# thomasneff/AdaNeRF

Measured on AMD Instinct MI355X. Metric: FPS at 800x800, higher is better.
Workload: dtype bf16

## Files before the change

### adanerf_amd/csrc/adanerf_hip.hip

```cpp
#include "../../include/adanerf_hip.h"

#include <hip/hip_runtime.h>

#include <sys/stat.h>

#include <algorithm>
#include <type_traits>
#include <cmath>
#include <cstdio>
#include <cstring>
#include <exception>
#include <string>
#include <vector>

#include "format.hpp"
#include "kernels.hip.hpp"
#include "launch_f32.hpp"
#include "k_generic_f32.hip.hpp"
#include "k_generic16.hip.hpp"
#include "pack.hpp"

using namespace adanerf;

namespace {
// ... 76 lines not shown
  int sample16_grid = 0;
  int sampling_mode = 0;
  DevBuf overflow;
  int sample_grid = 0;
  PackedDev net1[3];
  TensorMap net1_host;
  DevBuf ztab;
  bool coarse_fine = false;
  int n_coarse = 0;
  PackedDev netc[3];
  NetTopology topoc;
  bool genericc = false;
  GenericTopo genc{};
  ShadeParams spc{};
  DevBuf ztab_coarse, raw_coarse, key_coarse;
  int shade_gen_grid_c = 0;

  int cap_rays = 0, cap_nmax = 0;
  DevBuf rays, oracle, ray_offsets, ray_counts, selbin, selw, block_total, block_offset, total;
  DevBuf sample_key, sample_w, raw, sample_z;
  DevBuf guard_mask, refine_list, guard_probe;
  float guard_eps = 0.f;
  float guard_eps_pair = 0.f;
  int guard_audit_period = 0;
  DepthMap dm{};
  int shade_grid[3] = {0, 0, 0};
  int device = 0;
  float* aux_depth = nullptr;
  float* aux_acc = nullptr;
  float* aux_disp = nullptr;
  DevBuf disp_scratch;
  hipEvent_t peer_event = nullptr;
  uint64_t peer_tried = 0;
};

namespace {

#define HIP_TRY(ctx, expr)                                                                  \
  do {                                                                                      \
    hipError_t e_ = (expr);                                                                 \
    if (e_ != hipSuccess) {                                                                 \
      (ctx)->err = std::string(#expr) + ": " + hipGetErrorString(e_);                       \
      return ADANERF_EDEVICE;                                                               \
    }                                                                                       \
  } while (0)

#define BIND(ctx) HIP_TRY(ctx, hipSetDevice((ctx)->device))

int fail(adanerf_ctx* c, int code, const std::string& msg) {
  if (c) c->err = msg;
  else g_create_error = msg;
  return code;
}

int dev_alloc(adanerf_ctx* c, DevBuf* b, size_t bytes) {
  if (b->bytes >= bytes && b->p) return ADANERF_OK;
  if (b->p) HIP_TRY(c, hipFree(b->p));
  b->p = nullptr;
  b->bytes = 0;
  if (bytes == 0) return ADANERF_OK;
  HIP_TRY(c, hipMalloc(&b->p, bytes));
  b->bytes = bytes;
  return ADANERF_OK;
}

void dev_free(DevBuf* b) {
  if (b->p) (void)hipFree(b->p);
  b->p = nullptr;
  b->bytes = 0;
}

int upload_net(adanerf_ctx* c, const PackedNet& pn, PackedDev* d) {
  int rc;
  if ((rc = dev_alloc(c, &d->w, pn.weights.size()))) return rc;
  if ((rc = dev_alloc(c, &d->b, pn.bias.size() * sizeof(float)))) return rc;
  HIP_TRY(c, hipMemcpy(d->w.p, pn.weights.data(), pn.weights.size(), hipMemcpyHostToDevice));
  HIP_TRY(c, hipMemcpy(d->b.p, pn.bias.data(), pn.bias.size() * sizeof(float), hipMemcpyHostToDevice));
  d->params.w = reinterpret_cast<const u32x4*>(d->w.p);
  d->params.bias = reinterpret_cast<const float*>(d->b.p);
  for (size_t i = 0; i < pn.w_off.size() && i < kMaxLayers; ++i) {
// ... 381 lines not shown
template <typename K>
int occupancy_grid(adanerf_ctx* c, K kernel, int threads, int* out) {
  int per_cu = 0;
  HIP_TRY(c, hipOccupancyMaxActiveBlocksPerMultiprocessor(&per_cu, kernel, threads, 0));
  if (per_cu < 1) per_cu = 1;
  *out = per_cu * c->info.compute_units;
  return ADANERF_OK;
}

int calibrate_guard(adanerf_ctx* c, int n_poses, uint32_t seed, bool install, float* max_diff, float* max_pair);
int ensure_guard_band(adanerf_ctx* c);

bool has_split_sampling(const adanerf_ctx* c) { return (!c->generic0 || c->ray_samples == 0) && c->topo0.width != kWideWidth; }

bool generic_split_sampling(const adanerf_ctx* c) {
  return c->generic0 && c->sampling_mode != ADANERF_SAMPLING_FP32 && c->ray_samples == 0 && c->net0_split.w.p != nullptr;
}

int launch_sample_mlp(adanerf_ctx* c, int first_ray, int n_rays, float* d_oracle, float* d_rays, const SelectOut* sel = nullptr) {
  if (n_rays <= 0) return ADANERF_OK;
  SampleArgs a{};
  if (sel) {
    a.sel = *sel;
    a.fused_select = 1;
  }
  a.g = c->rg;
  a.net = c->net0.params;
  a.net16 = c->net0_split.params;
  a.overflow_flag = reinterpret_cast<int32_t*>(c->overflow.p);
  a.first_ray = first_ray;
  a.n_rays = n_rays;
  a.oracle_out = d_oracle;
  a.rays_out = d_rays;
  dim3 grid((n_rays + 127) / 128), block(256);
  const bool full = c->fp0 == 10 && c->fd0 == 4;
  if (c->generic0) {
    if (generic_split_sampling(c)) {
      const uint32_t bias_cap = c->topo0.width == 64 ? gen_bias_cap<64>() : c->topo0.width == 128 ? gen_bias_cap<128>() : gen_bias_cap<256>();
      if (tune::kGenericStaged && a.net16.n_bias > bias_cap)
        return fail(c, ADANERF_EUNSUPPORTED, "sampling network: bias table exceeds the kernel's LDS capacity");
#define ADN_GENS(FPv, FDv, Wv) hipLaunchKernelGGL((sample_mlp16x3_gen_kernel<FPv, FDv, Wv, tune::kGenericStaged>), grid, block, 0, c->stream, a, c->gen0)
#define ADN_GENS_W(FPv, FDv)                                   \
  do {                                                         \
    if (c->topo0.width == 64) ADN_GENS(FPv, FDv, 64);          \
    else if (c->topo0.width == 128) ADN_GENS(FPv, FDv, 128);   \
    else ADN_GENS(FPv, FDv, 256);                              \
  } while (0)
      if (c->enc0 == kEnc10_4) ADN_GENS_W(10, 4);
      else if (c->enc0 == kEnc2_2) ADN_GENS_W(2, 2);
      else ADN_GENS_W(kMaxBands, kMaxBands);
#undef ADN_GENS_W
#undef ADN_GENS
      HIP_TRY(c, hipGetLastError());
      return ADANERF_OK;
    }
    if (sel) return fail(c, ADANERF_EINVAL, "fused selection is not available on the fp32 run-time-shaped sampling kernel");
    HIP_TRY(c, launch_sample_mlp_gen(a, c->gen0, c->enc0, c->topo0.width, grid.x, c->stream));
    return ADANERF_OK;
  }
  const bool guarded = c->sampling_mode == ADANERF_SAMPLING_GUARDED && sel != nullptr;
  if (guarded) {
    if (!(c->guard_eps > 0.f)) {
      int rc = ensure_guard_band(c);
      if (rc) return rc;
    }
    a.sel.guard_mask = reinterpret_cast<uint32_t*>(c->guard_mask.p);
// ... 1 lines not shown
    a.sel.guard_pair = guard_pair_of(c->transform, c->guard_eps, c->guard_eps_pair);
    a.sel.audit_period = c->guard_audit_period;
    a.sel.audit_phase = c->guard_audit_period > 0 ? static_cast<int32_t>(c->guard_frame & static_cast<uint32_t>(c->guard_audit_period - 1)) : 0;
    a.sel.guard_probe = reinterpret_cast<float*>(c->guard_probe.p);
    a.sel.guard_rows = reinterpret_cast<float*>(c->oracle.p);
    if (c->debug_guard & 1) a.sel.guard_rows = nullptr;
    a.sel.guard_seen = reinterpret_cast<uint32_t*>(c->total.p) + 8;
  }
  if (c->sampling_mode == 1) {
    HIP_TRY(c, launch_sample_mlp_f32(a, full, grid.x, c->stream));
  } else if (c->sampling_mode == 2 || guarded) {
    if (!c->net0_f16.w.p) {
      PackedNet pn;
      std::string err;
      const NetShape sh = shape_of(c->fp0, c->fd0, c->fp1, c->fd1, c->ray_samples);
      if (!pack_sampling_net(c->net0_host, sh, Elem::F16, &pn, &err)) return fail(c, ADANERF_EIO, "model0.onnx: " + err);
      int rc = upload_net(c, pn, &c->net0_f16);
      if (rc) return rc;
    }
    a.net16 = c->net0_f16.params;
    if (!c->sample16_grid) {
      int rc = full ? occupancy_grid(c, sample_mlp16_kernel<10, 4>, 512, &c->sample16_grid)
                    : occupancy_grid(c, sample_mlp16_kernel<2, 2>, 512, &c->sample16_grid);
      if (rc) return rc;
    }
    const bool two_blocks = sel != nullptr && a.fused_select && !a.oracle_out && !(c->debug_guard & 2) && (n_rays >= kSample16x2MinRays || (c->debug_guard & 4));
    if (two_blocks) {
      if (!c->sample16x2_grid) {
        int rc = full ? occupancy_grid(c, sample_mlp16x2_kernel<10, 4>, 256, &c->sample16x2_grid)
                      : occupancy_grid(c, sample_mlp16x2_kernel<2, 2>, 256, &c->sample16x2_grid);
        if (rc) return rc;
      }
      dim3 g2(std::min<unsigned>((n_rays + 255) / 256, static_cast<unsigned>(c->sample16x2_grid))), b2(256);
      if (full) hipLaunchKernelGGL((sample_mlp16x2_kernel<10, 4>), g2, b2, 0, c->stream, a);
      else hipLaunchKernelGGL((sample_mlp16x2_kernel<2, 2>), g2, b2, 0, c->stream, a);
    } else {
    dim3 g16(std::min<unsigned>((n_rays + 255) / 256, static_cast<unsigned>(c->sample16_grid))), b16(512);
    if (full) hipLaunchKernelGGL((sample_mlp16_kernel<10, 4>), g16, b16, 0, c->stream, a);
    else hipLaunchKernelGGL((sample_mlp16_kernel<2, 2>), g16, b16, 0, c->stream, a);
    }
    if (guarded) {
      const int n_words = (n_rays + 31) / 32;
      int32_t* n_list = reinterpret_cast<int32_t*>(c->total.p) + 4;
      if (!c->sample_grid) {
        int rc = full ? occupancy_grid(c, sample_mlp16x3_kernel<10, 4>, 256, &c->sample_grid)
                      : occupancy_grid(c, sample_mlp16x3_kernel<2, 2>, 256, &c->sample_grid);
        if (rc) return rc;
      }
      const dim3 rgrid(std::min<unsigned>(grid.x, static_cast<unsigned>(c->sample_grid)));
      const int cap_round = (c->opt.flags & ADANERF_FLAG_GUARD_AUDIT_FILL) ? static_cast<int>(rgrid.x) * 128 : 0;
      const int cycle = a.sel.audit_period > 0 ? static_cast<int>((c->guard_frame / static_cast<uint32_t>(a.sel.audit_period)) & 0x7fffffffu) : 0;
      hipLaunchKernelGGL(refine_list_kernel, dim3((n_words + 255) / 256), dim3(256), 0, c->stream, reinterpret_cast<const uint32_t*>(c->guard_mask.p),
                         n_words, n_rays, a.sel.audit_period, a.sel.audit_phase, cap_round, cycle, reinterpret_cast<int32_t*>(c->refine_list.p), n_list);
      SampleArgs r = a;
      r.net16 = c->net0_split.params;
      r.rays_out = nullptr;
      r.sel.guard_mask = nullptr;
      r.sel.guard_band = c->guard_eps;
      r.sel.guard_band_pair = c->transform == kOracleRaw ? a.sel.guard_pair : 0.f;
      r.sel.guard_eps = 0.f;
      r.sel.guard_pair = 0.f;
      r.sel.audit_period = 0;
      r.sel.refine_list = reinterpret_cast<const int32_t*>(c->refine_list.p);
      r.ray_list = r.sel.refine_list;
      r.n_list = n_list;
      if (full) hipLaunchKernelGGL((sample_mlp16x3_kernel<10, 4>), rgrid, block, 0, c->stream, r);
      else hipLaunchKernelGGL((sample_mlp16x3_kernel<2, 2>), rgrid, block, 0, c->stream, r);
    }
  } else {
    if (!c->sample_grid) {
      int rc = full ? occupancy_grid(c, sample_mlp16x3_kernel<10, 4>, 256, &c->sample_grid)
                    : occupancy_grid(c, sample_mlp16x3_kernel<2, 2>, 256, &c->sample_grid);
      if (rc) return rc;
    }
    grid.x = std::min<unsigned>(grid.x, static_cast<unsigned>(c->sample_grid));
    if (full) hipLaunchKernelGGL((sample_mlp16x3_kernel<10, 4>), grid, block, 0, c->stream, a);
    else hipLaunchKernelGGL((sample_mlp16x3_kernel<2, 2>), grid, block, 0, c->stream, a);
  }
  HIP_TRY(c, hipGetLastError());
  return ADANERF_OK;
}

constexpr int kInlineScanMaxBlocks = 65536;

SelectOut select_out(adanerf_ctx* c, int n_max, float thr, int32_t* d_cnt) {
  SelectOut so{};
  so.counts = d_cnt;
  so.selbin = reinterpret_cast<uint8_t*>(c->selbin.p);
  so.selw = reinterpret_cast<float*>(c->selw.p);
  so.seg_total = reinterpret_cast<int32_t*>(c->block_total.p);
  so.n_max = n_max;
  so.thr = thr;
  so.transform = c->transform;
  return so;
}

int launch_expand(adanerf_ctx* c, int n_rays, int n_max, int seg_shift, int32_t* d_off, const int32_t* d_cnt, uint32_t* d_key, float* d_w,
                  int32_t* d_total) {
// ... 249 lines not shown
  return done(ADANERF_OK);
}

int ensure_guard_band(adanerf_ctx* c) {
  GuardRecord r;
  if (!(c->opt.flags & ADANERF_FLAG_NO_GUARD_CACHE) && read_guard_record(c, &r) && r.poses >= ADANERF_GUARD_CALIB_POSES) {
    install_guard_band(c, r.max_diff, r.max_pair, r.poses, ADANERF_GUARD_FROM_RECORD);
    return ADANERF_OK;
  }
  float d = 0.f, dp = 0.f;
  return calibrate_guard(c, ADANERF_GUARD_CALIB_POSES, 1u, true, &d, &dp);
}

constexpr int kShadeWaves = 8;

int launch_shade_mlp(adanerf_ctx* c, const float* d_rays, const uint32_t* d_key, const int32_t* d_total, int max_samples, int prec,
                     float* d_raw, const float* d_z = nullptr, bool coarse = false) {
  if (max_samples <= 0) return ADANERF_OK;
  const bool generic = coarse ? c->genericc : c->generic1;
  const NetTopology& topo = coarse ? c->topoc : c->topo1;
  const GenericTopo& gen = coarse ? c->genc : c->gen1;
  int& gen_grid = coarse ? c->shade_gen_grid_c : c->shade_gen_grid;
  int rc = coarse ? ensure_netc(c, prec) : ensure_net1(c, prec);
  if (rc) return rc;
  ShadeArgs a{};
  a.sp = coarse ? c->spc : c->sp;
  a.net = coarse ? c->netc[prec].params : c->net1[prec].params;
  a.rays = d_rays;
  a.sample_key = d_key;
  a.sample_z = d_z;
  a.total = d_total;
  a.max_samples = max_samples;
  a.raw_out = d_raw;
  if (generic && prec != ADANERF_PREC_FP32) {
    const int enc = coarse ? enc_layout(c->fp0, c->fd0, false) : c->enc1;
    const bool st = tune::kGenericStaged;
    const bool enc104 = enc == kEnc10_4;
    const int nb_wg = !st ? 1 : topo.width == 64 ? gen_blocks<64>() : topo.width == 128 ? (enc104 ? gen_blocks<128, 10>() : gen_blocks<128, kMaxBands>())
                                : topo.width == 256 ? gen_blocks<256>() : gen_blocks<512>();
    const int per_wg = 128 * nb_wg;
    const int tiles = (max_samples + per_wg - 1) / per_wg;
    const uint32_t bias_cap = topo.width == 64 ? gen_bias_cap<64>() : topo.width == 128 ? gen_bias_cap<128>()
                              : topo.width == 256 ? gen_bias_cap<256>() : gen_bias_cap<512>();
    if (st && a.net.n_bias > bias_cap)
      return fail(c, ADANERF_EUNSUPPORTED, "shading network: bias table exceeds the kernel's LDS capacity");
    int& grid16 = c->shade_gen16_grid[coarse ? 1 : 0][prec == ADANERF_PREC_BF16 ? 0 : 1];
#define ADN_GEN16_GO(KERNEL)                                                                                             \
  do {                                                                                                                   \
    if (!grid16) {                                                                                                       \
      int per_cu = 0;                                                                                                    \
      HIP_TRY(c, hipOccupancyMaxActiveBlocksPerMultiprocessor(&per_cu, KERNEL, 256, 0));                                 \
      grid16 = (per_cu < 1 ? 1 : per_cu) * c->info.compute_units;                                                        \
    }                                                                                                                    \
    hipLaunchKernelGGL(KERNEL, dim3(std::min(tiles, grid16)), dim3(256), 0, c->stream, a, gen);                          \
  } while (0)
#define ADN_GEN16(ET, FPv, FDv, Wv)                                                                                      \
  do {                                                                                                                   \
    if constexpr (tune::kGenericStaged)                                                                                  \
      ADN_GEN16_GO((shade_mlp16_gen_staged_kernel<ET, FPv, FDv, Wv, gen_blocks<Wv, FPv>(), gen_occupancy<Wv, FPv>()>));       \
    else ADN_GEN16_GO((shade_mlp16_gen_kernel<ET, FPv, FDv, Wv>));                                                       \
  } while (0)
#define ADN_GEN16_W(ET, FPv, FDv)                                  \
  do {                                                             \
    if (topo.width == 64) ADN_GEN16(ET, FPv, FDv, 64);             \
    else if (topo.width == 128) ADN_GEN16(ET, FPv, FDv, 128);      \
    else if (topo.width == 256) ADN_GEN16(ET, FPv, FDv, 256);      \
// ... 198 lines not shown
  c->guard_eps = opt->guard_eps > 0.f ? opt->guard_eps : 0.f;
  c->guard_eps_pair = (c->guard_eps > 0.f && opt->guard_eps_pair > 0.f) ? std::min(opt->guard_eps_pair, 2.0f * c->guard_eps) : 2.0f * c->guard_eps;
  c->guard_audit_period = opt->guard_audit_period == 0 ? ADANERF_GUARD_AUDIT_PERIOD : std::max(opt->guard_audit_period, 0);
  c->info.guard_eps = c->guard_eps;
  c->info.guard_eps_pair = c->guard_eps_pair;
  c->info.guard_audit_period = c->sampling_mode == ADANERF_SAMPLING_GUARDED ? c->guard_audit_period : 0;
  c->info.guard_calib_source = c->guard_eps > 0.f ? ADANERF_GUARD_FROM_OPTIONS : ADANERF_GUARD_FROM_NONE;
  if (c->sampling_mode == ADANERF_SAMPLING_GUARDED) c->model0_hash = fnv1a64_file(join_path(model_dir, "model0.onnx"));
  {
    PackedNet probe;
    if (!pack_shading_net(c->net1_host, sh, Elem::F32, &probe, &err)) return bail(ADANERF_EIO, "model1.onnx: " + err);
    c->topo1 = probe.topo;
    c->generic1 = !probe.topo.is_default(true) || c->enc1 == kEncMax;
    if (opt->precision == ADANERF_PREC_FP32) p1 = std::move(probe);
    else if (!pack_shading_net(c->net1_host, sh, elem_of(opt->precision), &p1, &err)) return bail(ADANERF_EIO, "model1.onnx: " + err);
  }
  auto width_ok = [](int w) { return w == 64 || w == 128 || w == 256 || w == kWideWidth; };
  if (c->genericc && !width_ok(c->topoc.width)) return bail(ADANERF_EUNSUPPORTED, "model0.onnx: layer width " + std::to_string(c->topoc.width) + " (64, 128, 256 or 512 supported)");
  if (c->generic0 && !width_ok(c->topo0.width)) return bail(ADANERF_EUNSUPPORTED, "model0.onnx: layer width " + std::to_string(c->topo0.width) + " (64, 128, 256 or 512 supported)");
  if (c->generic1 && !width_ok(c->topo1.width)) return bail(ADANERF_EUNSUPPORTED, "model1.onnx: layer width " + std::to_string(c->topo1.width) + " (64, 128, 256 or 512 supported)");

  int n_dev = 0;
  if (hipGetDeviceCount(&n_dev) != hipSuccess || n_dev <= 0)
    return bail(ADANERF_EDEVICE, "no HIP device available: libadanerf_hip has no CPU fallback");
  if (hipSetDevice(opt->device_id) != hipSuccess) return bail(ADANERF_EDEVICE, "hipSetDevice failed");
  hipDeviceProp_t prop;
  if (hipGetDeviceProperties(&prop, opt->device_id) != hipSuccess) return bail(ADANERF_EDEVICE, "hipGetDeviceProperties failed");
  if (std::string(prop.gcnArchName).find("gfx950") == std::string::npos)
    return bail(ADANERF_EDEVICE, std::string("device is ") + prop.gcnArchName + "; this library is built for gfx950 (MI355X) only");
  c->info.compute_units = prop.multiProcessorCount;
  c->device = opt->device_id;
  if (hipStreamCreateWithFlags(&c->own_stream, hipStreamNonBlocking) != hipSuccess) return bail(ADANERF_EDEVICE, "hipStreamCreate failed");
  c->stream = c->own_stream;

  rc = dev_alloc(c, &c->ztab, kBins * sizeof(float));
  if (rc) return bail(rc, c->err);
  if (hipMemcpy(c->ztab.p, ms.ztab.data(), kBins * sizeof(float), hipMemcpyHostToDevice) != hipSuccess)
    return bail(ADANERF_EDEVICE, "ztab upload failed");
  c->sp.ztab = reinterpret_cast<const float*>(c->ztab.p);
  if (c->coarse_fine) {
    if ((rc = upload_net(c, p0, &c->netc[opt->precision]))) return bail(rc, c->err);
    if ((rc = dev_alloc(c, &c->ztab_coarse, kMaxCoarse * sizeof(float)))) return bail(rc, c->err);
    if (hipMemcpy(c->ztab_coarse.p, ms.ztab_coarse.data(), ms.ztab_coarse.size() * sizeof(float), hipMemcpyHostToDevice) != hipSuccess)
      return bail(ADANERF_EDEVICE, "coarse depth table upload failed");
    c->spc = c->sp;
    c->spc.normalize = ms.normalize0;
    c->sp.unit_dir = 0;
    c->spc.ztab = reinterpret_cast<const float*>(c->ztab_coarse.p);
    c->genc = GenericTopo{c->topoc.depth, c->topoc.cat_mask, 0, 0, nullptr, 0.f};
  } else {
    if ((rc = upload_net(c, p0, &c->net0))) return bail(rc, c->err);
    if (has_split_sampling(c) && (rc = upload_net(c, p0s, &c->net0_split))) return bail(rc, c->err);
  }
  if (c->ray_samples > 0) {
    if ((rc = dev_alloc(c, &c->rsi_z, ms.rsi_z.size() * sizeof(float)))) return bail(rc, c->err);
    if (hipMemcpy(c->rsi_z.p, ms.rsi_z.data(), ms.rsi_z.size() * sizeof(float), hipMemcpyHostToDevice) != hipSuccess)
      return bail(ADANERF_EDEVICE, "raySampleInput depth table upload failed");
  }
  c->gen0 = GenericTopo{c->topo0.depth, 0, c->ray_samples, p0.rsi_w_off, reinterpret_cast<const float*>(c->rsi_z.p), c->cfg.depthRange[1]};
  c->gen1 = GenericTopo{c->topo1.depth, c->topo1.cat_mask, 0, 0, nullptr, 0.f};
  if ((rc = dev_alloc(c, &c->overflow, 64))) return bail(rc, c->err);
  if (hipMemset(c->overflow.p, 0, 64) != hipSuccess) return bail(ADANERF_EDEVICE, "hipMemset failed");
  if ((rc = upload_net(c, p1, &c->net1[opt->precision]))) return bail(rc, c->err);
  if ((rc = ensure_batch_buffers(c, c->info.batch_rays, c->info.num_samples))) return bail(rc, c->err);
  *out = c;
  return ADANERF_OK;
// ... 70 lines not shown
      layer_out[4 * i + 1] = pn.topo.ray_samples;
      layer_out[4 * i + 2] = pe_slots(sh.lp0 ? sh.lp0 : sh.fp0);
      layer_out[4 * i + 3] = pn.mtiles[0];
    }
    if (scaled) {
      const size_t i = pn.w_off.size();
      layer_out[4 * i + 0] = pn.out_exp[0];
      layer_out[4 * i + 1] = pn.out_exp[1];
      layer_out[4 * i + 2] = 0;
      layer_out[4 * i + 3] = -1;
    }
  }
  *weights_bytes = pn.weights.size();
  *bias_floats = pn.bias.size();
  *n_layers = n_rec;
  return ADANERF_OK;
} catch (const std::exception& e) {
  return fail(nullptr, ADANERF_EIO, std::string("adanerf_host_pack_weights: ") + e.what());
}

int adanerf_destroy(adanerf_ctx* c) {
  if (!c) return ADANERF_OK;
  (void)hipSetDevice(c->device);
  if (c->peer_event) (void)hipEventDestroy(c->peer_event);
  if (c->stream) (void)hipStreamSynchronize(c->stream);
  for (hipEvent_t e : c->events) (void)hipEventDestroy(e);
  for (int32_t* p : c->pinned_totals) (void)hipHostFree(p);
  if (c->guard_host) (void)hipHostFree(c->guard_host);
  if (c->guard_ev) (void)hipEventDestroy(c->guard_ev);
  DevBuf* bufs[] = {&c->net0_split.w, &c->net0_split.b, &c->net0_f16.w, &c->net0_f16.b, &c->overflow, &c->net0.w, &c->net0.b, &c->net1[0].w, &c->net1[0].b, &c->net1[1].w, &c->net1[1].b, &c->net1[2].w, &c->net1[2].b,
                    &c->ztab, &c->rays, &c->oracle, &c->ray_offsets, &c->ray_counts, &c->selbin, &c->selw, &c->block_total,
                    &c->block_offset, &c->total, &c->sample_key, &c->sample_w, &c->raw, &c->sample_z, &c->rsi_z,
                    &c->netc[0].w, &c->netc[0].b, &c->netc[1].w, &c->netc[1].b, &c->netc[2].w, &c->netc[2].b, &c->ztab_coarse, &c->raw_coarse, &c->key_coarse,
                    &c->guard_mask, &c->refine_list, &c->guard_probe, &c->disp_scratch};
  for (DevBuf* b : bufs) dev_free(b);
  if (c->own_stream) (void)hipStreamDestroy(c->own_stream);
  delete c;
  return ADANERF_OK;
}

int adanerf_get_info(const adanerf_ctx* c, adanerf_info* info) {
  if (!c || !info) return ADANERF_EINVAL;
  *info = c->info;
  return ADANERF_OK;
}

int adanerf_set_camera(adanerf_ctx* c, const float pos[3], const float rot[9]) {
  if (!c) return ADANERF_EINVAL;
  if (!pos || !rot) return fail(c, ADANERF_EINVAL, "pos/rot == NULL");
  if (c->pos_bound.active) {
    double d2 = 0.0;
    for (int i = 0; i < 3; ++i) d2 += (pos[i] - c->pos_bound.center[i]) * (pos[i] - c->pos_bound.center[i]);
    const double bound = c->pos_bound.at(std::sqrt(d2));
    if (!(bound <= kPosIdentityBound)) {
      char msg[256];
      std::snprintf(msg, sizeof(msg), "camera %.3g away from the view-cell centre: sample positions can reach %.3g, beyond the %.0f the bf16 shading path's "
                    "layer scaling assumes -- create the context with precision fp16 or fp32 for such poses", std::sqrt(d2), bound, kPosIdentityBound);
      return fail(c, ADANERF_EUNSUPPORTED, msg);
    }
  }
  std::memcpy(c->rg.pos, pos, 3 * sizeof(float));
  std::memcpy(c->rg.rot, rot, 9 * sizeof(float));
  return ADANERF_OK;
}

int adanerf_sync(adanerf_ctx* c) {
  if (!c) return ADANERF_EINVAL;
// ... 626 lines not shown
```

### adanerf_amd/csrc/k_mlp16.hip.hpp

```cpp
#pragma once
#include "k_common.hip.hpp"
#include "k_mlp_f32.hip.hpp"
#include "tuning.hpp"
#include <utility>

namespace adanerf {


struct ShadeArgs {
  ShadeParams sp;
  NetParams net;
  const float* rays;
  const uint32_t* sample_key;
  const float* sample_z;
  const int32_t* total;
  int32_t max_samples;
  float* raw_out;
};

__device__ __forceinline__ void store_raw(const ShadeArgs& a, int s, float r, float g, float b, float alpha) {
  const float ks = a.net.out_scale[1];
  *reinterpret_cast<float4*>(a.raw_out + static_cast<size_t>(s) * 4) = make_float4(r * ks, g * ks, b * ks, alpha * a.net.out_scale[0]);
}

struct Bf16 {
  static constexpr bool kClampRelu = true;
  typedef bf16x8 vec8;
  static __device__ __forceinline__ uint32_t pack(float lo, float hi) {
    f32x2 v = {lo, hi};
    return __builtin_bit_cast(uint32_t, __builtin_convertvector(v, bf16x2));
  }
  static __device__ __forceinline__ f32x16 mfma(u32x4 a, u32x4 b, f32x16 c) {
    return __builtin_amdgcn_mfma_f32_32x32x16_bf16(__builtin_bit_cast(bf16x8, a), __builtin_bit_cast(bf16x8, b), c, 0, 0, 0);
  }
};
struct Fp16 {
  static constexpr bool kClampRelu = false;
  typedef f16x8 vec8;
  static __device__ __forceinline__ uint32_t pack(float lo, float hi) {
    f32x2 v = {lo, hi};
    return __builtin_bit_cast(uint32_t, __builtin_convertvector(v, f16x2));
  }
  static __device__ __forceinline__ f32x16 mfma(u32x4 a, u32x4 b, f32x16 c) {
    return __builtin_amdgcn_mfma_f32_32x32x16_f16(__builtin_bit_cast(f16x8, a), __builtin_bit_cast(f16x8, b), c, 0, 0, 0);
  }
};

using tune::kRegFrags;
constexpr int kShadeFrags16 = 32 + 4 * 128 + 160 + 2 * 128 + 144 + 72 + 8;
constexpr int kShadeBiasFloats = 8 * 256 + 288 + 128 + 32;
// ... 496 lines not shown
      if (CARRY_OUT && kCarry) {
        pend.a = accA;
        pend.b = accB;
      } else {
        gA = mfma_guard<ET, RELU>(accA);
        gB = mfma_guard<ET, RELU>(accB);
#pragma unroll
        for (int g = 0; g < 4; ++g) epilogue_quad_16<ET, RELU>(accA, m, g, outA, gA);
#pragma unroll
        for (int g = 0; g < 4; ++g) epilogue_quad_16<ET, RELU>(accB, m, g, outB, gB);
      }
    }
  }
}

template <class ET, int FP, int FD>
__global__ __launch_bounds__(256) void shade_mlp16x2_kernel(ShadeArgs a) {
  static_assert(FP == 10 && FD == 4, "fragment positions below assume the 10-4 shading encoding");
  constexpr int QP = pe_slots(FP), QD = pe_slots(FD);
  constexpr int WAVES = 4, TILE = WAVES * 64, CF = tune::kChunkFrags2, RS = tune::kRingSlots2, LPW = CF / WAVES;
  constexpr int kRingBytes = CF * RS * 1024;
  static_assert(CF % WAVES == 0 && CF % tune::kRegFrags2 == 0 && kShadeFrags16 % CF == 0 && CF % 8 == 0 && CF <= 32, "chunk geometry");
  typedef WStream<CF, RS, LPW, tune::kRegFrags2> WS;
  constexpr int kStashPerBlock = (QP / 8 + QD / 8) * 1024;
  __shared__ __attribute__((aligned(16))) char lds[kRingBytes + kShadeBiasFloats * 4 + WAVES * 2 * kStashPerBlock];
  const int lane = lane_id();
  const int wave = __builtin_amdgcn_readfirstlane(static_cast<int>(threadIdx.x) >> 6);
  const int j = lane & 31, h = lane >> 5;
  const uint32_t stash = static_cast<uint32_t>(reinterpret_cast<uintptr_t>(lds)) + kRingBytes + kShadeBiasFloats * 4 +
                         wave * 2 * kStashPerBlock + lane * 16;
  int total = a.total ? *a.total : a.max_samples;
  if (total > a.max_samples) total = a.max_samples;
  const int ntiles = (total + TILE - 1) / TILE;
  if (static_cast<int>(blockIdx.x) >= ntiles) return;
  {
    float* lds_bias = reinterpret_cast<float*>(lds + kRingBytes);
    for (int i = threadIdx.x; i < kShadeBiasFloats; i += blockDim.x) lds_bias[i] = a.net.bias[i];
  }
  __syncthreads();
  WS st;
  ws_start(st, a.net.w, kShadeFrags16 * 1024, lds, wave, lane);
  const uint32_t bias0 = static_cast<uint32_t>(reinterpret_cast<uintptr_t>(lds)) + kRingBytes + h * 64;
  const uint32_t* bo = a.net.b_off;
  for (int tile = blockIdx.x; tile < ntiles; tile += gridDim.x) {
    const int s0 = tile * TILE + wave * 64 + j, s1 = s0 + 32;
    uint32_t hA0[64], hB0[64], hA1[64], hB1[64];
    PendingTile2 pend;
    {
      float x[3], dpe[3];
      uint32_t pts0[QP / 2], pts1[QP / 2], dirs[QD / 2];
      load_sample(a, s0, total, x, dpe);
      pe_pack<ET, FP>(x, h, pts0);
      pe_pack<ET, FD>(dpe, h, dirs);
      lds_stash_write<QP / 8>(stash, pts0);
      lds_stash_write<QD / 8>(stash + (QP / 8) * 1024, dirs);
      load_sample(a, s1, total, x, dpe);
      pe_pack<ET, FP>(x, h, pts1);
      pe_pack<ET, FD>(dpe, h, dirs);
      lds_stash_write<QP / 8>(stash + kStashPerBlock, pts1);
      lds_stash_write<QD / 8>(stash + kStashPerBlock + (QP / 8) * 1024, dirs);
      layer_16x2<ET, WS, QP / 8, 0, 8, true, 0, -1, -1, true, true>(st, bias0 + bo[0] * 4, pts0, pts0, pts1, pts1, hA0, hA1, pend);
    }
#pragma unroll 1
    for (int l = 1; l <= 3; l += 2) {
      layer_16x2<ET, WS, 16, 0, 8, true, 0, -1, 7, true, true>(st, bias0 + bo[l] * 4, hA0, hA0, hA1, hA1, hB0, hB1, pend, hA0, hA1);
      layer_16x2<ET, WS, 16, 0, 8, true, 0, -1, 7, true, true>(st, bias0 + bo[l + 1] * 4, hB0, hB0, hB1, hB1, hA0, hA1, pend, hB0, hB1);
    }
    {
      uint32_t pts0[QP / 2], pts1[QP / 2];
      lds_stash_read<QP / 8>(stash, pts0);
      lds_stash_read<QP / 8>(stash + kStashPerBlock, pts1);
      layer_16x2<ET, WS, QP / 8, 16, 8, true, 0, -1, 7, true, true>(st, bias0 + bo[5] * 4, pts0, hA0, pts1, hA1, hB0, hB1, pend, hA0, hA1);
    }
    layer_16x2<ET, WS, 16, 0, 8, true, 0, -1, 7, true, true>(st, bias0 + bo[6] * 4, hB0, hB0, hB1, hB1, hA0, hA1, pend, hB0, hB1);
    layer_16x2<ET, WS, 16, 0, 8, true, 0, -1, 7, true, true>(st, bias0 + bo[7] * 4, hA0, hA0, hA1, hA1, hB0, hB1, pend, hA0, hA1);
    f32x16 alpha0, alpha1;
    layer_16x2<ET, WS, 16, 0, 9, false, 0, 8, 7, true, false>(st, bias0 + bo[8] * 4, hB0, hB0, hB1, hB1, hA0, hA1, pend, hB0, hB1, &alpha0, &alpha1);
    {
      uint32_t d0[QD / 2], d1[QD / 2];
      lds_stash_read<QD / 8>(stash + (QP / 8) * 1024, d0);
      lds_stash_read<QD / 8>(stash + kStashPerBlock + (QP / 8) * 1024, d1);
      layer_16x2<ET, WS, 16, QD / 8, 4, true, (32 + 4 * 128 + 160 + 2 * 128 + 144) % CF>(st, bias0 + bo[9] * 4, hA0, d0, hA1, d1, hB0, hB1, pend);
    }
    f32x16 rgb0, rgb1;
    layer_16x2<ET, WS, 8, 0, 1, false, (32 + 4 * 128 + 160 + 2 * 128 + 144 + 72) % CF, 0>(st, bias0 + bo[10] * 4, hB0, hB0, hB1, hB1, hA0, hA1, pend, nullptr, nullptr, &rgb0, &rgb1);
    if (h == 0 && s0 < total)
      store_raw(a, s0, rgb0[0], rgb0[1], rgb0[2], alpha0[0]);
    if (h == 0 && s1 < total)
      store_raw(a, s1, rgb1[0], rgb1[1], rgb1[2], alpha1[0]);
  }
  asm volatile("s_waitcnt vmcnt(0)" ::: "memory");
}

template <int FP, int FD>
__global__ __launch_bounds__(256) void shade_mlp32_kernel(ShadeArgs a) {
  constexpr int QP = pe_slots(FP), QD = pe_slots(FD);
  constexpr int TILE = 4 * 32;
  const int lane = lane_id();
  const int wave = __builtin_amdgcn_readfirstlane(static_cast<int>(threadIdx.x) >> 6);
  const int j = lane & 31, h = lane >> 5;
  int total = a.total ? *a.total : a.max_samples;
  if (total > a.max_samples) total = a.max_samples;
  const u32x4* w = a.net.w;
  const float* b = a.net.bias;

  for (int tile = blockIdx.x; tile * TILE < total; tile += gridDim.x) {
    const int s = tile * TILE + wave * 32 + j;
    if (tile * TILE + wave * 32 >= total) continue;
    asm volatile("" : "+v"(w), "+v"(b));
    float x[3], dpe[3];
    load_sample(a, s, total, x, dpe);
    float pts[QP], dirs[QD], hA[144], hB[128];
    pe_eval<FP, true>(x, h, pts);
    pe_eval<FD, true>(dpe, h, dirs);
    layer_f32<QP, 0, 8, true>(w + a.net.w_off[0], b + a.net.b_off[0], lane, pts, pts, hA);
#pragma unroll 1
    for (int l = 1; l <= 3; l += 2) {
      layer_f32<128, 0, 8, true>(w + a.net.w_off[l], b + a.net.b_off[l], lane, hA, hA, hB);
      layer_f32<128, 0, 8, true>(w + a.net.w_off[l + 1], b + a.net.b_off[l + 1], lane, hB, hB, hA);
    }
    layer_f32<QP, 128, 8, true>(w + a.net.w_off[5], b + a.net.b_off[5], lane, pts, hA, hB);
    layer_f32<128, 0, 8, true>(w + a.net.w_off[6], b + a.net.b_off[6], lane, hB, hB, hA);
    layer_f32<128, 0, 8, true>(w + a.net.w_off[7], b + a.net.b_off[7], lane, hA, hA, hB);
// ... 39 lines not shown
```

### adanerf_amd/csrc/k_mlp_f32.hip.hpp

```cpp
#pragma once
#include "k_common.hip.hpp"
#include "k_select_pair.hip.hpp"

namespace adanerf {


template <int Q1, int Q2, int MT, bool RELU>
__device__ __forceinline__ void layer_f32(const u32x4* __restrict__ w, const float* __restrict__ bias, int lane,
                                          const float* in1, const float* in2, float* out) {
  constexpr int QS = Q1 + Q2;
  static_assert(Q1 % 4 == 0 && Q2 % 4 == 0, "fp32 engine groups 4 k-steps per 16-byte fragment");
  const int h = lane >> 5;
#pragma unroll
  for (int m = 0; m < MT; ++m) {
    f32x16 acc;
    const float4* bp = reinterpret_cast<const float4*>(bias + (m * 2 + h) * 16);
#pragma unroll
    for (int g = 0; g < 4; ++g) {
      float4 b = bp[g];
      acc[4 * g + 0] = b.x;
      acc[4 * g + 1] = b.y;
      acc[4 * g + 2] = b.z;
      acc[4 * g + 3] = b.w;
    }
#pragma unroll
    for (int s4 = 0; s4 < QS / 4; ++s4) {
      const f32x4 a = reinterpret_cast<const f32x4*>(w)[(m * (QS / 4) + s4) * 64 + lane];
      const float* in = (4 * s4 < Q1) ? (in1 + 4 * s4) : (in2 + (4 * s4 - Q1));
      acc = __builtin_amdgcn_mfma_f32_32x32x2f32(a[0], in[0], acc, 0, 0, 0);
      acc = __builtin_amdgcn_mfma_f32_32x32x2f32(a[1], in[1], acc, 0, 0, 0);
      acc = __builtin_amdgcn_mfma_f32_32x32x2f32(a[2], in[2], acc, 0, 0, 0);
      acc = __builtin_amdgcn_mfma_f32_32x32x2f32(a[3], in[3], acc, 0, 0, 0);
    }
#pragma unroll
    for (int r = 0; r < 16; ++r) out[16 * m + r] = RELU ? fmaxf(acc[r], 0.f) : acc[r];
  }
}

struct SampleArgs {
  RayGenParams g;
  NetParams net;
  NetParams net16;
  int32_t* overflow_flag;
  int32_t first_ray, n_rays;
  float* oracle_out;
  float* rays_out;
  SelectOut sel;
  int32_t fused_select;
  const int32_t* ray_list;
  const int32_t* n_list;
};

template <int FP, int FD>
__global__ __launch_bounds__(256) void sample_mlp_kernel(SampleArgs a) {
  const int lane = lane_id();
  const int wave = __builtin_amdgcn_readfirstlane(static_cast<int>(threadIdx.x) >> 6);
  const int j = lane & 31, h = lane >> 5;
  const int blk = blockIdx.x * 4 + wave;
  if (blk * 32 >= a.n_rays) return;
  const int local = blk * 32 + j;
  const bool valid = local < a.n_rays;
  const int ray = a.first_ray + (valid ? local : a.n_rays - 1);

  int col, row;
  ray_pixel(a.g, ray, &col, &row);
  float nds[3], p[3], u[3];
  gen_ray(a.g, col, row, nds, p);
  unit3(nds, u);

  constexpr int QD = pe_slots(FD), QP = pe_slots(FP), Q0 = QD + QP;
  float bufA[128], bufB[128];
  pe_eval<FD, true>(u, h, bufA);
  pe_eval<FP, true>(p, h, bufA + QD);

  const u32x4* w = a.net.w;
  const float* b = a.net.bias;
  layer_f32<Q0, 0, 8, true>(w + a.net.w_off[0], b + a.net.b_off[0], lane, bufA, bufA, bufB);
#pragma unroll 1
  for (int l = 1; l <= 5; l += 2) {
    layer_f32<128, 0, 8, true>(w + a.net.w_off[l], b + a.net.b_off[l], lane, bufB, bufB, bufA);
    layer_f32<128, 0, 8, true>(w + a.net.w_off[l + 1], b + a.net.b_off[l + 1], lane, bufA, bufA, bufB);
  }
  layer_f32<128, 0, 4, false>(w + a.net.w_off[7], b + a.net.b_off[7], lane, bufB, bufB, bufA);
// ... 77 lines not shown
```

### adanerf_amd/csrc/k_sampling16.hip.hpp

```cpp
#pragma once
#include "k_mlp16.hip.hpp"

namespace adanerf {



__device__ __forceinline__ void split_pack(float v0, float v1, uint32_t* hi, uint32_t* lo) {
  const f32x2 v = {v0, v1};
  const f16x2 h = __builtin_convertvector(v, f16x2);
  *hi = __builtin_bit_cast(uint32_t, h);
  const f32x2 r = {(v0 - static_cast<float>(h[0])) * kSplitScale, (v1 - static_cast<float>(h[1])) * kSplitScale};
  *lo = __builtin_bit_cast(uint32_t, __builtin_convertvector(r, f16x2));
}

template <bool LAST>
__device__ __forceinline__ void epilogue_pair_16x3(const f32x16& acc, const f32x16& cross, int m, int pi, uint32_t* out_hi,
                                                   uint32_t* out_lo, float* out_f32) {
  float v0 = __builtin_fmaf(cross[2 * pi], 1.0f / kSplitScale, acc[2 * pi]);
  float v1 = __builtin_fmaf(cross[2 * pi + 1], 1.0f / kSplitScale, acc[2 * pi + 1]);
  if (LAST) {
    out_f32[16 * m + 2 * pi] = v0;
    out_f32[16 * m + 2 * pi + 1] = v1;
  } else {
    split_pack(relu_bits(v0), relu_bits(v1), &out_hi[8 * m + pi], &out_lo[8 * m + pi]);
// ... 75 lines not shown
      for (int g = 0; g < 8; ++g) asm volatile("" : "=v"(out_hi[8 * m + g]), "=v"(out_lo[8 * m + g]));
      continue;
    }
    if (PIPE && m + 1 < MT) {
      pacc = acc;
      pcross = cross;
    } else if (CARRY && !LAST) {
      static_assert(LAST || !tune::kSplitCarry || MT == 8, "the carried tile is tile 7");
      pend.acc = acc;
      pend.cross = cross;
    } else {
#pragma unroll
      for (int pi = 0; pi < 8; ++pi) epilogue_pair_16x3<LAST>(acc, cross, m, pi, out_hi, out_lo, out_f32);
    }
  }
}

template <int FP, int FD>
__global__ __launch_bounds__(256) void sample_mlp16x3_kernel(SampleArgs a) {
  constexpr int QD = pe_slots(FD), QP = pe_slots(FP), Q0 = QD + QP;
  constexpr int WAVES = 4, CF = tune::kChunkFragsSampling, RS = tune::kRingSlotsSampling, LPW = CF / WAVES, TILE = WAVES * 32;
  constexpr int F0 = 2 * (Q0 / 8) * 8;
  constexpr int FRAGS = F0 + 6 * 256 + 128;
  static_assert(F0 % CF == 0 && FRAGS % CF == 0 && CF % WAVES == 0 && CF % tune::kRegFragsSampling == 0 && CF <= 32, "chunk geometry");
  typedef WStream<CF, RS, LPW, tune::kRegFragsSampling> WS;
  constexpr int kRingBytes = CF * RS * 1024, kBiasFloats = 7 * 256 + 128;
  __shared__ __attribute__((aligned(16))) char lds[kRingBytes + kBiasFloats * 4 + WAVES * kPairLdsBytesPerWave];
  const int lane = lane_id();
  const int wave = __builtin_amdgcn_readfirstlane(static_cast<int>(threadIdx.x) >> 6);
  const int j = lane & 31, h = lane >> 5;
  int n_rays = a.n_rays;
  if (a.ray_list) n_rays = min(n_rays, __builtin_amdgcn_readfirstlane(*a.n_list));
  const int ntiles = (n_rays + TILE - 1) / TILE;
  if (static_cast<int>(blockIdx.x) >= ntiles) return;
  const uint32_t sel_stage = static_cast<uint32_t>(reinterpret_cast<uintptr_t>(lds)) + kRingBytes + kBiasFloats * 4 +
                             wave * kPairLdsBytesPerWave + lane * 16;

  {
    float* lds_bias = reinterpret_cast<float*>(lds + kRingBytes);
    for (int i = threadIdx.x; i < kBiasFloats; i += blockDim.x) lds_bias[i] = a.net16.bias[i];
  }
  __syncthreads();
  WS st;
  ws_start(st, a.net16.w, FRAGS * 1024, lds, wave, lane);
  const uint32_t bias0 = static_cast<uint32_t>(reinterpret_cast<uintptr_t>(lds)) + kRingBytes + h * 64;
  const uint32_t* bo = a.net16.b_off;

  GuardAcc gacc;
  for (int tile = blockIdx.x; tile < ntiles; tile += gridDim.x) {
    const int local = tile * TILE + wave * 32 + j;
    const bool valid = local < n_rays;
    const int lidx = valid ? local : n_rays - 1;
    const int entry = a.ray_list ? a.ray_list[lidx] : 0;
    const int ray = a.first_ray + (a.ray_list ? (entry & kRefineRayMask) : lidx);
    int col, row;
    ray_pixel(a.g, ray, &col, &row);
    float nds[3], p[3], u[3];
    gen_ray(a.g, col, row, nds, p);
    unit3(nds, u);

    uint32_t aH[64], aL[64], bH[64], bL[64];
    if (tune::kAblateSample & 256) {
#pragma unroll
      for (int q = 0; q < Q0 / 2; ++q) {
        aH[q] = __builtin_bit_cast(uint32_t, u[q % 3]) >> 3;
        aL[q] = __builtin_bit_cast(uint32_t, p[q % 3]) >> 5;
      }
    } else {
      float t[Q0];
      pe_eval<FD, !(tune::kAblateSample & 128)>(u, h, t);
      pe_eval<FP, !(tune::kAblateSample & 128)>(p, h, t + QD);
#pragma unroll
      for (int q = 0; q < Q0 / 2; ++q) split_pack(t[2 * q], t[2 * q + 1], &aH[q], &aL[q]);
    }
    PendingTile3 pend;
    layer_16x3<WS, Q0 / 8, 8, false, 0, false>(st, bias0 + bo[0] * 4, lane, aH, aL, bH, bL, nullptr, pend);
#pragma unroll 1
    for (int l = 1; l <= 5; l += 2) {
      layer_16x3<WS, 16, 8, false, 0, true>(st, bias0 + bo[l] * 4, lane, bH, bL, aH, aL, nullptr, pend);
      layer_16x3<WS, 16, 8, false, 0, true>(st, bias0 + bo[l + 1] * 4, lane, aH, aL, bH, bL, nullptr, pend);
    }
    float out[64];
// ... 6 lines not shown
      const bool bad_ray = (z != z) | (pair_xchg(static_cast<uint32_t>(z != z)) != 0u);
      if (bad_ray && valid && h == 0 && a.overflow_flag) atomicAdd(a.overflow_flag, 1);
      if (tune::kAblateSample & 512) {
        if (valid && h == 0) a.sel.counts[local] = 1 + (__builtin_bit_cast(int, out[0] + out[17] + out[35] + out[63]) & 3);
        if (lane == 0 && valid) a.sel.seg_total[local >> kPairSegShift] = 64;
      } else {
        pair_epilogue(out, lane, local, valid, sel_stage, a.sel, false, entry, &gacc);
      }
    }
    if (valid) {
      if (a.oracle_out) {
        float* o = a.oracle_out + static_cast<size_t>(local) * kBins;
        bool bad = false;
#pragma unroll
        for (int m = 0; m < 4; ++m)
#pragma unroll
          for (int g = 0; g < 4; ++g) {
            float4 v = make_float4(out[16 * m + 4 * g], out[16 * m + 4 * g + 1], out[16 * m + 4 * g + 2], out[16 * m + 4 * g + 3]);
            bad |= !(fabsf(v.x) < 3.0e38f) | !(fabsf(v.y) < 3.0e38f) | !(fabsf(v.z) < 3.0e38f) | !(fabsf(v.w) < 3.0e38f);
            *reinterpret_cast<float4*>(o + 32 * m + 8 * g + 4 * h) = v;
          }
        const bool bad_ray = bad | (pair_xchg(static_cast<uint32_t>(bad)) != 0u);
        if (bad_ray && h == 0 && a.overflow_flag) atomicAdd(a.overflow_flag, 1);
      }
      if (a.rays_out) {
        float ro[3] = {p[0], p[1], p[2]}, rd[3] = {nds[0], nds[1], nds[2]};
        if (a.g.use_ndc) ndc_ray(a.g, p, nds, ro, rd);
        float4* r = reinterpret_cast<float4*>(a.rays_out + static_cast<size_t>(local) * 8);
        if (h == 0) r[0] = make_float4(ro[0], ro[1], ro[2], 0.f);
        else r[1] = make_float4(rd[0], rd[1], rd[2], 0.f);
      }
    }
  }
  if (a.fused_select && a.ray_list) guard_flush(a.sel, gacc, lane);
  asm volatile("s_waitcnt vmcnt(0)" ::: "memory");
}

constexpr int kGuardEngineRev = 4;

template <int FP, int FD>
constexpr int sample16_frags() { return ((pe_slots(FD) + pe_slots(FP)) / 8) * 8 + 6 * 128 + 64; }

template <int FP, int FD>
__global__ __launch_bounds__(512, 2) void sample_mlp16_kernel(SampleArgs a) {
  constexpr int QD = pe_slots(FD), QP = pe_slots(FP), Q0 = QD + QP;
  constexpr bool kOneGroupDma = tune::kDmaGroup >= 0;
  constexpr int WAVES = 8, CF = 16, RS = 4, LPW = kOneGroupDma ? CF / 4 : CF / WAVES, TILE = WAVES * 32;
  constexpr int F0 = (Q0 / 8) * 8, FRAGS = sample16_frags<FP, FD>();
  static_assert(F0 % CF == 0 && FRAGS % CF == 0 && CF % WAVES == 0 && CF % kRegFrags == 0 && CF <= 32, "chunk geometry");
  typedef WStream<CF, RS, LPW> WS;
  constexpr int kRingBytes = CF * RS * 1024, kBiasFloats = 7 * 256 + 128;
  __shared__ __attribute__((aligned(16))) char lds[kRingBytes + kBiasFloats * 4 + WAVES * kPairLdsBytesPerWave];
  const int lane = lane_id();
  const int wave = __builtin_amdgcn_readfirstlane(static_cast<int>(threadIdx.x) >> 6);
  const int j = lane & 31, h = lane >> 5;
  const int WT = (a.n_rays + 31) >> 5, G = static_cast<int>(gridDim.x);
  const int q = WT / (WAVES * G), rem = WT - WAVES * G * q, k = (rem + G - 1) / G;
  const bool has_partial = static_cast<int>(blockIdx.x) * k < rem;
  const int rounds = q + (has_partial ? 1 : 0);
  if (rounds == 0) return;
  const uint32_t sel_stage = static_cast<uint32_t>(reinterpret_cast<uintptr_t>(lds)) + kRingBytes + kBiasFloats * 4 +
                             wave * kPairLdsBytesPerWave + lane * 16;
  {
    float* lds_bias = reinterpret_cast<float*>(lds + kRingBytes);
    for (int i = threadIdx.x; i < kBiasFloats; i += blockDim.x) lds_bias[i] = a.net16.bias[i];
  }
// ... 66 lines not shown
    if (valid && a.oracle_out) {
      float* o = a.oracle_out + static_cast<size_t>(local) * kBins;
      bool bad = false;
#pragma unroll
      for (int m = 0; m < 4; ++m)
#pragma unroll
        for (int g = 0; g < 4; ++g) {
          const float4 v = make_float4(out[m][4 * g], out[m][4 * g + 1], out[m][4 * g + 2], out[m][4 * g + 3]);
          bad |= !(fabsf(v.x) < 3.0e38f) | !(fabsf(v.y) < 3.0e38f) | !(fabsf(v.z) < 3.0e38f) | !(fabsf(v.w) < 3.0e38f);
          *reinterpret_cast<float4*>(o + 32 * m + 8 * g + 4 * h) = v;
        }
      const bool bad_ray = bad | (pair_xchg(static_cast<uint32_t>(bad)) != 0u);
      if (bad_ray && h == 0 && a.overflow_flag) atomicAdd(a.overflow_flag, 1);
    }
  }
  asm volatile("s_waitcnt vmcnt(0)" ::: "memory");
}

constexpr int kSample16x2MinRays = 4 * 256 * 256;

template <int FP, int FD>
__global__ __launch_bounds__(256) void sample_mlp16x2_kernel(SampleArgs a) {
  constexpr int QD = pe_slots(FD), QP = pe_slots(FP), Q0 = QD + QP;
  constexpr int WAVES = 4, CF = 16, RS = 6, LPW = CF / WAVES, TILE = WAVES * 64;
  constexpr int F0 = (Q0 / 8) * 8, FRAGS = sample16_frags<FP, FD>();
  static_assert(F0 % CF == 0 && FRAGS % CF == 0 && CF % tune::kRegFrags2 == 0, "chunk geometry");
  typedef WStream<CF, RS, LPW, tune::kRegFrags2> WS;
  constexpr int kRingBytes = CF * RS * 1024, kBiasFloats = 7 * 256 + 128;
  __shared__ __attribute__((aligned(16))) char lds[kRingBytes + kBiasFloats * 4 + WAVES * kPairLdsBytesPerWave];
  const int lane = lane_id();
  const int wave = __builtin_amdgcn_readfirstlane(static_cast<int>(threadIdx.x) >> 6);
  const int j = lane & 31, h = lane >> 5;
  const int ntiles = (a.n_rays + TILE - 1) / TILE;
  if (static_cast<int>(blockIdx.x) >= ntiles) return;
  const uint32_t sel_stage = static_cast<uint32_t>(reinterpret_cast<uintptr_t>(lds)) + kRingBytes + kBiasFloats * 4 +
                             wave * kPairLdsBytesPerWave + lane * 16;
  {
    float* lds_bias = reinterpret_cast<float*>(lds + kRingBytes);
    for (int i = threadIdx.x; i < kBiasFloats; i += blockDim.x) lds_bias[i] = a.net16.bias[i];
  }
  __syncthreads();
  WS st;
  ws_start(st, a.net16.w, FRAGS * 1024, lds, wave, lane);
  const uint32_t bias0 = static_cast<uint32_t>(reinterpret_cast<uintptr_t>(lds)) + kRingBytes + h * 64;
  const uint32_t* bo = a.net16.b_off;

  for (int tile = blockIdx.x; tile < ntiles; tile += gridDim.x) {
    uint32_t hA0[64], hB0[64], hA1[64], hB1[64];
    PendingTile2 pend;
    int local[2];
    bool valid[2];
    {
      uint32_t in0[2][Q0 / 2];
#pragma unroll
      for (int b = 0; b < 2; ++b) {
        local[b] = tile * TILE + wave * 64 + 32 * b + j;
        valid[b] = local[b] < a.n_rays;
        const int ray = a.first_ray + (valid[b] ? local[b] : a.n_rays - 1);
        int col, row;
        ray_pixel(a.g, ray, &col, &row);
        float nds[3], p[3], u[3];
        gen_ray(a.g, col, row, nds, p);
        unit3(nds, u);
        if (valid[b] && a.rays_out) {
          float ro[3] = {p[0], p[1], p[2]}, rd[3] = {nds[0], nds[1], nds[2]};
          if (a.g.use_ndc) ndc_ray(a.g, p, nds, ro, rd);
          float4* r = reinterpret_cast<float4*>(a.rays_out + static_cast<size_t>(local[b]) * 8);
          if (h == 0) r[0] = make_float4(ro[0], ro[1], ro[2], 0.f);
          else r[1] = make_float4(rd[0], rd[1], rd[2], 0.f);
        }
        float t[Q0];
        pe_eval<FD, !tune::kFastPeFp16Pass>(u, h, t);
        pe_eval<FP, !tune::kFastPeFp16Pass>(p, h, t + QD);
#pragma unroll
        for (int q = 0; q < Q0 / 2; ++q) in0[b][q] = Fp16::pack(t[2 * q], t[2 * q + 1]);
      }
      layer_16x2<Fp16, WS, Q0 / 8, 0, 8, true, 0, -1, -1, true, true>(st, bias0 + bo[0] * 4, in0[0], in0[0], in0[1], in0[1], hA0, hA1, pend);
    }
#pragma unroll 1
    for (int l = 1; l <= 5; l += 2) {
      layer_16x2<Fp16, WS, 16, 0, 8, true, 0, -1, 7, true, true>(st, bias0 + bo[l] * 4, hA0, hA0, hA1, hA1, hB0, hB1, pend, hA0, hA1);
      layer_16x2<Fp16, WS, 16, 0, 8, true, 0, -1, 7, true, true>(st, bias0 + bo[l + 1] * 4, hB0, hB0, hB1, hB1, hA0, hA1, pend, hB0, hB1);
    }
    f32x16 outA[4], outB[4];
    layer_16x2<Fp16, WS, 16, 0, 4, false, 0, kKeepAllF32, 7, true, false>(st, bias0 + bo[7] * 4, hA0, hA0, hA1, hA1, hB0, hB1, pend, hA0, hA1, outA, outB);
#pragma unroll
    for (int b = 0; b < 2; ++b) {
      float x[64];
      float z = 0.f;
#pragma unroll
      for (int i = 0; i < 64; ++i) {
        x[i] = b ? outB[i >> 4][i & 15] : outA[i >> 4][i & 15];
        z = __builtin_fmaf(x[i], 0.f, z);
      }
      const bool bad_ray = (z != z) | (pair_xchg(static_cast<uint32_t>(z != z)) != 0u);
      if (bad_ray && valid[b] && h == 0 && a.overflow_flag && !a.sel.guard_mask) atomicAdd(a.overflow_flag, 1);
      pair_epilogue<false>(x, lane, local[b], valid[b], sel_stage, a.sel, bad_ray);
    }
  }
  asm volatile("s_waitcnt vmcnt(0)" ::: "memory");
}

}
```

Before: 218.9.

## Replace static grid-stride tile loop with atomic dynamic tile claiming

Persistent MLP kernels (sampling x2/x3 and shading) now fetch their next tile from a global atomic counter instead of striding by gridDim. The claim is issued early in each tile and waited on through a vmcnt threshold, so it overlaps with the weight-streaming loads. The last block to finish resets the counters. The aim is to balance load across persistent blocks with uneven per-tile cost. In exchange it adds a per-tile barrier and atomic traffic, and it relies on hand-written inline asm with fragile vmcnt assumptions.

```diff
diff --git a/adanerf_amd/csrc/adanerf_hip.hip b/adanerf_amd/csrc/adanerf_hip.hip
--- a/adanerf_amd/csrc/adanerf_hip.hip
+++ b/adanerf_amd/csrc/adanerf_hip.hip
@@ -132,6 +132,7 @@
   DevBuf disp_scratch;
   hipEvent_t peer_event = nullptr;
   uint64_t peer_tried = 0;
+  DevBuf tiles;
 };
 
 namespace {
@@ -146,6 +147,8 @@
   } while (0)
 
 #define BIND(ctx) HIP_TRY(ctx, hipSetDevice((ctx)->device))
+
+int32_t* tile_counters(adanerf_ctx* c) { return reinterpret_cast<int32_t*>(c->tiles.p); }
 
 int fail(adanerf_ctx* c, int code, const std::string& msg) {
   if (c) c->err = msg;
@@ -593,6 +596,7 @@
   a.n_rays = n_rays;
   a.oracle_out = d_oracle;
   a.rays_out = d_rays;
+  a.tiles = tile_counters(c);
   dim3 grid((n_rays + 127) / 128), block(256);
   const bool full = c->fp0 == 10 && c->fd0 == 4;
   if (c->generic0) {
@@ -660,6 +664,7 @@
         if (rc) return rc;
       }
       dim3 g2(std::min<unsigned>((n_rays + 255) / 256, static_cast<unsigned>(c->sample16x2_grid))), b2(256);
+      a.tiles = tile_counters(c);
       if (full) hipLaunchKernelGGL((sample_mlp16x2_kernel<10, 4>), g2, b2, 0, c->stream, a);
       else hipLaunchKernelGGL((sample_mlp16x2_kernel<2, 2>), g2, b2, 0, c->stream, a);
     } else {
@@ -692,6 +697,7 @@
       r.sel.refine_list = reinterpret_cast<const int32_t*>(c->refine_list.p);
       r.ray_list = r.sel.refine_list;
       r.n_list = n_list;
+      r.tiles = tile_counters(c);
       if (full) hipLaunchKernelGGL((sample_mlp16x3_kernel<10, 4>), rgrid, block, 0, c->stream, r);
       else hipLaunchKernelGGL((sample_mlp16x3_kernel<2, 2>), rgrid, block, 0, c->stream, r);
     }
@@ -1007,6 +1013,7 @@
   a.total = d_total;
   a.max_samples = max_samples;
   a.raw_out = d_raw;
+  a.tiles = tile_counters(c);
   if (generic && prec != ADANERF_PREC_FP32) {
     const int enc = coarse ? enc_layout(c->fp0, c->fd0, false) : c->enc1;
     const bool st = tune::kGenericStaged;
@@ -1271,6 +1278,9 @@
   c->device = opt->device_id;
   if (hipStreamCreateWithFlags(&c->own_stream, hipStreamNonBlocking) != hipSuccess) return bail(ADANERF_EDEVICE, "hipStreamCreate failed");
   c->stream = c->own_stream;
+  rc = dev_alloc(c, &c->tiles, 2 * sizeof(int32_t));
+  if (rc) return bail(rc, c->err);
+  if (hipMemsetAsync(c->tiles.p, 0, c->tiles.bytes, c->stream) != hipSuccess) return bail(ADANERF_EDEVICE, "tile counters: hipMemsetAsync failed");
 
   rc = dev_alloc(c, &c->ztab, kBins * sizeof(float));
   if (rc) return bail(rc, c->err);
@@ -1407,7 +1417,7 @@
                     &c->ztab, &c->rays, &c->oracle, &c->ray_offsets, &c->ray_counts, &c->selbin, &c->selw, &c->block_total,
                     &c->block_offset, &c->total, &c->sample_key, &c->sample_w, &c->raw, &c->sample_z, &c->rsi_z,
                     &c->netc[0].w, &c->netc[0].b, &c->netc[1].w, &c->netc[1].b, &c->netc[2].w, &c->netc[2].b, &c->ztab_coarse, &c->raw_coarse, &c->key_coarse,
-                    &c->guard_mask, &c->refine_list, &c->guard_probe, &c->disp_scratch};
+                    &c->guard_mask, &c->refine_list, &c->guard_probe, &c->disp_scratch, &c->tiles};
   for (DevBuf* b : bufs) dev_free(b);
   if (c->own_stream) (void)hipStreamDestroy(c->own_stream);
   delete c;
diff --git a/adanerf_amd/csrc/k_mlp16.hip.hpp b/adanerf_amd/csrc/k_mlp16.hip.hpp
--- a/adanerf_amd/csrc/k_mlp16.hip.hpp
+++ b/adanerf_amd/csrc/k_mlp16.hip.hpp
@@ -16,6 +16,35 @@
   const int32_t* total;
   int32_t max_samples;
   float* raw_out;
+  int32_t* tiles;
+};
+
+constexpr int kMinTileVmem = 64;
+struct TileClaim {
+  int32_t* ctr;
+  int* slot;
+  int pending = 0;
+  int parity = 0;
+  __device__ __forceinline__ void issue() {
+    if (threadIdx.x == 0)
+      asm volatile("s_nop 4\n\tglobal_atomic_add %0, %1, %2, %3 sc0   ; tile claim: issue" : "=a"(pending) : "v"(0), "a"(1), "s"(ctr) : "memory");
+  }
+  __device__ __forceinline__ int take() {
+    int* w = slot + parity;
+    parity ^= 1;
+    if (threadIdx.x == 0) {
+      asm volatile("s_waitcnt vmcnt(63)   ; tile claim: returned" : "+a"(pending) : : "memory");
+      *w = pending + static_cast<int>(gridDim.x);
+    }
+    asm volatile("s_waitcnt lgkmcnt(0)\n\ts_barrier   ; tile claim: published" ::: "memory");
+    return __builtin_amdgcn_readfirstlane(*w);
+  }
+  __device__ __forceinline__ void done() const {
+    if (threadIdx.x == 0 && atomicAdd(ctr + 1, 1) == static_cast<int>(gridDim.x) - 1) {
+      atomicExch(ctr, 0);
+      atomicExch(ctr + 1, 0);
+    }
+  }
 };
 
 __device__ __forceinline__ void store_raw(const ShadeArgs& a, int s, float r, float g, float b, float alpha) {
@@ -578,7 +607,13 @@
   int total = a.total ? *a.total : a.max_samples;
   if (total > a.max_samples) total = a.max_samples;
   const int ntiles = (total + TILE - 1) / TILE;
-  if (static_cast<int>(blockIdx.x) >= ntiles) return;
+  static_assert(kShadeFrags16 / WAVES >= kMinTileVmem, "TileClaim: a wave's weight copies per tile retire the claim (vmcnt(63))");
+  __shared__ int claim_words[2];
+  TileClaim claim{a.tiles, claim_words};
+  if (static_cast<int>(blockIdx.x) >= ntiles) {
+    claim.done();
+    return;
+  }
   {
     float* lds_bias = reinterpret_cast<float*>(lds + kRingBytes);
     for (int i = threadIdx.x; i < kShadeBiasFloats; i += blockDim.x) lds_bias[i] = a.net.bias[i];
@@ -588,7 +623,8 @@
   ws_start(st, a.net.w, kShadeFrags16 * 1024, lds, wave, lane);
   const uint32_t bias0 = static_cast<uint32_t>(reinterpret_cast<uintptr_t>(lds)) + kRingBytes + h * 64;
   const uint32_t* bo = a.net.b_off;
-  for (int tile = blockIdx.x; tile < ntiles; tile += gridDim.x) {
+  for (int tile = blockIdx.x; tile < ntiles; tile = claim.take()) {
+    claim.issue();
     const int s0 = tile * TILE + wave * 64 + j, s1 = s0 + 32;
     uint32_t hA0[64], hB0[64], hA1[64], hB1[64];
     PendingTile2 pend;
@@ -635,6 +671,7 @@
     if (h == 0 && s1 < total)
       store_raw(a, s1, rgb1[0], rgb1[1], rgb1[2], alpha1[0]);
   }
+  claim.done();
   asm volatile("s_waitcnt vmcnt(0)" ::: "memory");
 }
 
diff --git a/adanerf_amd/csrc/k_mlp_f32.hip.hpp b/adanerf_amd/csrc/k_mlp_f32.hip.hpp
--- a/adanerf_amd/csrc/k_mlp_f32.hip.hpp
+++ b/adanerf_amd/csrc/k_mlp_f32.hip.hpp
@@ -49,6 +49,7 @@
   int32_t fused_select;
   const int32_t* ray_list;
   const int32_t* n_list;
+  int32_t* tiles;
 };
 
 template <int FP, int FD>
diff --git a/adanerf_amd/csrc/k_sampling16.hip.hpp b/adanerf_amd/csrc/k_sampling16.hip.hpp
--- a/adanerf_amd/csrc/k_sampling16.hip.hpp
+++ b/adanerf_amd/csrc/k_sampling16.hip.hpp
@@ -131,7 +131,13 @@
   int n_rays = a.n_rays;
   if (a.ray_list) n_rays = min(n_rays, __builtin_amdgcn_readfirstlane(*a.n_list));
   const int ntiles = (n_rays + TILE - 1) / TILE;
-  if (static_cast<int>(blockIdx.x) >= ntiles) return;
+  static_assert(FRAGS / WAVES >= kMinTileVmem, "TileClaim: a wave's weight copies per tile retire the claim (vmcnt(63))");
+  __shared__ int claim_words[2];
+  TileClaim claim{a.tiles, claim_words};
+  if (static_cast<int>(blockIdx.x) >= ntiles) {
+    claim.done();
+    return;
+  }
   const uint32_t sel_stage = static_cast<uint32_t>(reinterpret_cast<uintptr_t>(lds)) + kRingBytes + kBiasFloats * 4 +
                              wave * kPairLdsBytesPerWave + lane * 16;
 
@@ -146,7 +152,8 @@
   const uint32_t* bo = a.net16.b_off;
 
   GuardAcc gacc;
-  for (int tile = blockIdx.x; tile < ntiles; tile += gridDim.x) {
+  for (int tile = blockIdx.x; tile < ntiles; tile = claim.take()) {
+    claim.issue();
     const int local = tile * TILE + wave * 32 + j;
     const bool valid = local < n_rays;
     const int lidx = valid ? local : n_rays - 1;
@@ -219,6 +226,7 @@
       }
     }
   }
+  claim.done();
   if (a.fused_select && a.ray_list) guard_flush(a.sel, gacc, lane);
   asm volatile("s_waitcnt vmcnt(0)" ::: "memory");
 }
@@ -351,7 +359,13 @@
   const int wave = __builtin_amdgcn_readfirstlane(static_cast<int>(threadIdx.x) >> 6);
   const int j = lane & 31, h = lane >> 5;
   const int ntiles = (a.n_rays + TILE - 1) / TILE;
-  if (static_cast<int>(blockIdx.x) >= ntiles) return;
+  static_assert(FRAGS / WAVES >= kMinTileVmem, "TileClaim: a wave's weight copies per tile retire the claim (vmcnt(63))");
+  __shared__ int claim_words[2];
+  TileClaim claim{a.tiles, claim_words};
+  if (static_cast<int>(blockIdx.x) >= ntiles) {
+    claim.done();
+    return;
+  }
   const uint32_t sel_stage = static_cast<uint32_t>(reinterpret_cast<uintptr_t>(lds)) + kRingBytes + kBiasFloats * 4 +
                              wave * kPairLdsBytesPerWave + lane * 16;
   {
@@ -364,7 +378,8 @@
   const uint32_t bias0 = static_cast<uint32_t>(reinterpret_cast<uintptr_t>(lds)) + kRingBytes + h * 64;
   const uint32_t* bo = a.net16.b_off;
 
-  for (int tile = blockIdx.x; tile < ntiles; tile += gridDim.x) {
+  for (int tile = blockIdx.x; tile < ntiles; tile = claim.take()) {
+    claim.issue();
     uint32_t hA0[64], hB0[64], hA1[64], hB1[64];
     PendingTile2 pend;
     int local[2];
@@ -417,6 +432,7 @@
       pair_epilogue<false>(x, lane, local[b], valid[b], sel_stage, a.sel, bad_ray);
     }
   }
+  claim.done();
   asm volatile("s_waitcnt vmcnt(0)" ::: "memory");
 }
 
```

New measurement: 223.1 (median of 6 runs). 1.02x the previous value.
